# ChenyangLEI/All-In-One-Deflicker

Hardware: NVIDIA H100
Metric: atlas_iters_per_sec (higher is better)
Workload: dtype fp32 (2-term fp16 split on wgmma, fp32 accumulate)

## Files before the change

all-in-one-deflicker_b200/csrc/mlp_tc.cu:

```cuda
#include <mutex>
#include <vector>

#include "tc_api.cuh"
#include "tc_ptx.cuh"
#include "loss_math.h"

namespace b200 {
using namespace ptx;

constexpr int TM = 128;
constexpr int HID = 256;
constexpr int ITEM_BYTES = 16384;
constexpr int CHUNK_BYTES = 4 * ITEM_BYTES;
constexpr float S_ACT = 16.0f;
constexpr float S_W = 256.0f;
constexpr int ATOM_BYTES = TM * 128;
constexpr int TILE_IMG_BYTES = 4 * ATOM_BYTES;
constexpr int PE_COLS = 40;

__host__ __device__ __forceinline__ int atom_off(int m, int k) {
  const int r = m & 7;
  return (m >> 3) * 1024 + r * 128 + (((k >> 3) ^ r) << 4) + ((k & 7) << 1);
}
__host__ __device__ __forceinline__ int item_off(int n, int k) {
// ... 209 lines not shown
                                              uint32_t& scale, int& pending, const Consumer& c) {
  consume_item<NST, NN>(pp, acc, a_hi, a_lo, true, scale, pending, c);
  consume_item<NST, NN>(pp, acc, a_hi + 64, a_lo + 64, true, scale, pending, c);
  consume_item<NST, NN>(pp, acc, a_hi, a_lo, false, scale, pending, c);
  consume_item<NST, NN>(pp, acc, a_hi + 64, a_lo + 64, false, scale, pending, c);
}
template <int NST, int R>
__device__ __forceinline__ void finish_pass(Pipe<NST>& pp, float (&acc)[R], int& pending, const Consumer& c) {
  wgmma_wait<0>();
  acc_fence(acc);
  if (pending >= 0 && c.warp_leader) mbar_arrive(&pp.empty[pending]);
  pending = -1;
}

__device__ __forceinline__ void store_tile_rows(const Consumer& c, const char* a_tile, char* g_img, int64_t term_stride) {
  if (!c.leader) return;
#pragma unroll
  for (int term = 0; term < 2; ++term)
#pragma unroll
    for (int j = 0; j < 4; ++j)
      bulk_s2g(g_img + term * term_stride + j * ATOM_BYTES + c.g * WG_ROW_BYTES,
               a_tile + term * TILE_IMG_BYTES + j * ATOM_BYTES + c.g * WG_ROW_BYTES, WG_ROW_BYTES);
  bulk_commit();
}
__device__ __forceinline__ void a_tile_reusable(const Consumer& c) {
  if (c.leader) bulk_wait_read0();
  c.sync();
}
__device__ __forceinline__ void a_tile_written(const Consumer& c) {
  fence_proxy_async_smem();
  c.sync();
}

__device__ __forceinline__ uint32_t relu_flag(float v) { return (uint32_t)(-(int)__float_as_uint(v)) >> 31; }

__device__ __forceinline__ uint32_t piece_bits(uint32_t f0, uint32_t f1, int col) {
  const int i = col & 15;
  uint32_t b = (f0 << (15 - i)) | (f1 << (14 - i));
  return b;
}
__device__ __forceinline__ uint32_t quad_or(uint32_t b) {
  b |= __shfl_xor_sync(0xffffffffu, b, 1);
  b |= __shfl_xor_sync(0xffffffffu, b, 2);
  return b;
}
__device__ __forceinline__ float quad_sum(float v) {
  v += __shfl_xor_sync(0xffffffffu, v, 1);
  return v + __shfl_xor_sync(0xffffffffu, v, 2);
}

constexpr int SMEM_A = 2 * TILE_IMG_BYTES;
constexpr int SMEM_AUX = 2 * ATOM_BYTES;
constexpr int RSUM_B_BYTES = 64 * 16;
constexpr int BWD_ACC_FLOATS = 5 * 256 + 768;
constexpr int SMEM_BWD_CONST_FLOATS = CONSUMER_WGS * (RSUM_B_BYTES / 4 + BWD_ACC_FLOATS);
constexpr int SMEM_BARS = 256;
constexpr int SMEM_MAX = 227 * 1024;
template <bool ATLAS, bool BWD> struct KCfg {
  static constexpr int NST = BWD ? 5 : (ATLAS ? 3 : 5);
  static constexpr int SMEM = SMEM_A + NST * ITEM_BYTES + (ATLAS && !BWD ? SMEM_AUX : 0) +
                              (BWD ? SMEM_BWD_CONST_FLOATS * 4 : FWD_CST_BYTES) + SMEM_BARS;
  static_assert(SMEM <= SMEM_MAX, "fused kernel exceeds the shared memory of one CTA");
  static_assert(SMEM + ITEM_BYTES > SMEM_MAX, "one more weight slot would fit");
  static_assert(2 * NST * 8 + 8 <= SMEM_BARS, "ring and constant barriers exceed their shared-memory slot");
};

template <int NST>
struct SmemMap {
  char* a_tile; char* stage; char* aux; float* cst;
  uint64_t* full; uint64_t* empty;
  __device__ __forceinline__ void init(char* raw, int aux_bytes, int cst_floats) {
    char* p = raw;
    a_tile = p; p += SMEM_A;
    stage = p; p += NST * ITEM_BYTES;
    aux = p; p += aux_bytes;
    cst = reinterpret_cast<float*>(p); p += cst_floats * 4;
    full = reinterpret_cast<uint64_t*>(p);
    empty = full + NST;
  }
};

template <int NST>
__device__ __forceinline__ void setup_cta(SmemMap<NST>& sm, bool cst_bar = false) {
  if (threadIdx.x == 0) {
    if (smem_u32(sm.a_tile) & 1023u) __trap();
    for (int i = 0; i < NST; ++i) { mbar_init(&sm.full[i], 1); mbar_init(&sm.empty[i], EMPTY_ARRIVALS); }
    if (cst_bar) mbar_init(&sm.empty[NST], 1);
    fence_barrier_init();
  }
  __syncthreads();
}
constexpr int BAR_CONSUMERS = 9;

struct FwdParams {
  const float* x;
  float* y;
  const float* params;
  int64_t w_off[B200_MAX_LAYERS], b_off[B200_MAX_LAYERS];
  NetImages img;
  int cap, n_groups; const int* n_valid;
  int g_fwd, g_bwd;
  float in_scale, in_shift;
  int store_images;
  int tanh_out;
  int pe_freqs;
};

template <bool ATLAS, int NL = (ATLAS ? 8 : 6), int VAR = 0>
__global__ void __launch_bounds__(TC_THREADS, 1) tc_fwd_kernel(const __grid_constant__ FwdParams P) {
  extern __shared__ __align__(1024) char smem_raw[];
  constexpr int NST = KCfg<ATLAS, false>::NST;
  SmemMap<NST> sm; sm.init(smem_raw, ATLAS ? SMEM_AUX : 0, FWD_CST_BYTES / 4);
  const int warp = warp_uniform(), lane = threadIdx.x & 31;
  constexpr int L = NL;
  constexpr int FIRST_TC = ATLAS ? 0 : 1;
  constexpr int LAST_TC = L - 2;
  constexpr bool PE3 = ATLAS && VAR > 0;
  constexpr bool SKIPS = ATLAS && !PE3;
  constexpr int OUT = ATLAS ? (PE3 ? VAR : 3) : 2;
  constexpr int KLAST = SKIPS ? 296 : 256;
  constexpr FwdConsts CST = fwd_consts(L, !ATLAS, OUT, KLAST);
  static_assert(CST.floats * 4 <= FWD_CST_BYTES, "forward constants exceed their shared-memory slot");
  uint64_t* cst_full = &sm.empty[NST];
  const int pe_cols = VAR == 1 ? 30 : 6 * P.pe_freqs;
  setup_cta(sm, true);
  TileIter ti; ti.init(P.cap, P.n_groups, P.n_valid, P.g_fwd, P.g_bwd);

  if (warp >= CONSUMER_WGS * 4) {
    setmaxnreg_dec<PRODUCER_REGS>();
    if (warp == CONSUMER_WGS * 4 && lane == 0) {
      mbar_expect_tx(cst_full, CST.floats * 4);
      bulk_g2s(sm.cst, P.img.cst, CST.floats * 4, cst_full);
      Pipe<NST> pp{sm.full, sm.empty, sm.stage, 0};
      for (int t = blockIdx.x; t < ti.total; t += gridDim.x)
        for (int l = FIRST_TC; l <= LAST_TC; ++l) {
          const char* base = P.img.w_fwd + P.img.w_fwd_layer[l];
          if (ATLAS && l == 0) { produce_items(pp, base, 4); continue; }
          if (SKIPS && l == 4) produce_items(pp, base + (int64_t)4 * CHUNK_BYTES, 4);
          produce_items(pp, base, 16);
        }
    }
    return;
  }
  setmaxnreg_inc<CONSUMER_REGS>();
  Consumer c; c.init();
  Pipe<NST> pp{sm.full, sm.empty, sm.stage, 0};
  int pending = -1;
  const float inv_scale = 1.0f / S_W;
  const float* wlast = sm.cst + CST.wl;
  const uint32_t a_rows = smem_u32(sm.a_tile) + c.g * WG_ROW_BYTES;
  const uint32_t aux_rows = smem_u32(sm.aux) + c.g * WG_ROW_BYTES;
  float acc[128];
  mbar_wait(cst_full, 0);
  for (int t = blockIdx.x; t < ti.total; t += gridDim.x) {
    const int gt = ti.global_tile(t);
    const int64_t row0 = (int64_t)gt * TM + c.m0;
    uint16_t* bits_row = reinterpret_cast<uint16_t*>(P.img.bits) + row0 * 16;
    auto put = [&](int m, int col, float v0, float v1) {
      uint32_t h, lo;
      split2_packed(v0, v1, h, lo);
      const int off = tile_off(m, col);
      *reinterpret_cast<uint32_t*>(sm.a_tile + off) = h;
      *reinterpret_cast<uint32_t*>(sm.a_tile + TILE_IMG_BYTES + off) = lo;
    };
    uint32_t held0 = 0, held1 = 0;
    auto flags_out = [&](int slot, int i, int col, uint32_t b0, uint32_t b1) {
      if ((i & 1) == 0) { held0 = b0; held1 = b1; return; }
      b0 = quad_or(b0 | held0); b1 = quad_or(b1 | held1);
      if (P.store_images && c.q == 0) {
        uint16_t* dst = bits_row + (int64_t)slot * P.img.rows * 16 + (col >> 4);
        dst[0] = (uint16_t)b0;
        dst[8 * 16] = (uint16_t)b1;
      }
    };
    auto bias_relu = [&](const float* bias, int i, int col, float (&v)[4]) {
      const float2 bs = *reinterpret_cast<const float2*>(bias + col);
      v[0] = fmaxf(__fmaf_rn(acc[4 * i], inv_scale, bs.x), 0.f);
      v[1] = fmaxf(__fmaf_rn(acc[4 * i + 1], inv_scale, bs.y), 0.f);
      v[2] = fmaxf(__fmaf_rn(acc[4 * i + 2], inv_scale, bs.x), 0.f);
      v[3] = fmaxf(__fmaf_rn(acc[4 * i + 3], inv_scale, bs.y), 0.f);
    };
    if (ATLAS) {
      c.sync();
      for (int task = c.tid; task < 64 * 8; task += 128) {
        const int m = 64 * c.g + (task & 63), c8 = task >> 6;
        const int64_t row = (int64_t)gt * TM + m;
        float in[3] = {0.f, 0.f, 0.f};
// ... 142 lines not shown
  if (c.leader) bulk_wait_all0();
}

struct BwdParams {
  const float* dy;
  const float* y;
  const float* x;
  float* d_in;
  const float* params;
  float* grads;
  int64_t w_off[B200_MAX_LAYERS], b_off[B200_MAX_LAYERS];
  NetImages img;
  int cap, n_groups; const int* n_valid;
  int* gmax_bits;
  int g_fwd, g_bwd;
  float in_scale;
  int d_in_accumulate;
  int tanh_out;
};

__device__ __forceinline__ void grad_scales(const int* gmax_bits, bool mapping, float& s_g, float& inv_sg) {
  const float mx = __int_as_float(gmax_bits[mapping ? 1 : 0]);
  int e = 0;
  if (mx > 0.f && mx < 3.0e38f) frexpf(mx, &e);
  e = max(-60, min(60, e));
  s_g = ldexpf(1.0f, 13 - e);
  inv_sg = ldexpf(1.0f, e - 13);
}

template <bool ATLAS, int NL = (ATLAS ? 8 : 6), int VAR = 0>
__global__ void __launch_bounds__(TC_THREADS, 1) tc_bwd_kernel(const __grid_constant__ BwdParams P) {
  extern __shared__ __align__(1024) char smem_raw[];
  constexpr int NST = KCfg<ATLAS, true>::NST;
  SmemMap<NST> sm; sm.init(smem_raw, 0, SMEM_BWD_CONST_FLOATS);
  const int warp = warp_uniform(), lane = threadIdx.x & 31;
  constexpr int L = NL;
  constexpr bool PE3 = ATLAS && VAR > 0;
  constexpr bool SKIPS = ATLAS && !PE3;
  constexpr int OUT = ATLAS ? (PE3 ? VAR : 3) : 2;
  constexpr int KLAST = SKIPS ? 296 : 256;
  constexpr int LOW = 1;
  constexpr bool HAS_DPE = ATLAS && !PE3;
  constexpr bool MAPPING = OUT == 2;
  static_assert((L - 1) * 256 + (ATLAS ? 0 : 768) <= BWD_ACC_FLOATS, "gradient accumulators exceed their slice");
  char* rsum_b = reinterpret_cast<char*>(sm.cst);
  float* s_acc = sm.cst + CONSUMER_WGS * RSUM_B_BYTES / 4;
  for (int i = threadIdx.x; i < CONSUMER_WGS * BWD_ACC_FLOATS; i += blockDim.x) s_acc[i] = 0.f;
  setup_cta(sm);
  TileIter ti; ti.init(P.cap, P.n_groups, P.n_valid, P.g_fwd, P.g_bwd);
  float s_g, inv_sg;
  grad_scales(P.gmax_bits, MAPPING, s_g, inv_sg);

  if (warp >= CONSUMER_WGS * 4) {
    setmaxnreg_dec<PRODUCER_REGS>();
    if (warp == CONSUMER_WGS * 4 && lane == 0) {
      Pipe<NST> pp{sm.full, sm.empty, sm.stage, 0};
      for (int t = blockIdx.x; t < ti.total; t += gridDim.x)
        for (int l = L - 2; l >= (HAS_DPE ? 0 : LOW); --l)
          produce_items(pp, P.img.w_bwd + P.img.w_bwd_layer[l], 16, l == 0 ? 64 * 64 : ITEM_BYTES);
    }
    return;
  }
  setmaxnreg_inc<CONSUMER_REGS>();
  Consumer c; c.init();
  Pipe<NST> pp{sm.full, sm.empty, sm.stage, 0};
  int pending = -1;
  const float inv_dgrad = inv_sg * (1.0f / S_W);
  const uint16_t* bits16 = reinterpret_cast<const uint16_t*>(P.img.bits);
  const float* wlast = P.params + P.w_off[L - 1];
  const uint32_t a_rows = smem_u32(sm.a_tile) + c.g * WG_ROW_BYTES;
  const uint32_t b_rows = smem_u32(rsum_b) + c.g * RSUM_B_BYTES;
  float* g_acc = s_acc + c.g * BWD_ACC_FLOATS;
  float acc[128];
  auto row_sums = [&](int slot) {
    float (&red)[16] = *reinterpret_cast<float(*)[16]>(&acc);
    uint32_t a_base = a_rows, b_base = b_rows;
    asm volatile("" : "+r"(a_base), "+r"(b_base));
    const uint64_t ad = make_desc(a_base, ATOM_BYTES, 1024), bd = make_desc_rows16(b_base);
    wgmma_fence();
#pragma unroll
    for (int blk = 0; blk < 4; ++blk)
#pragma unroll
      for (int ks = 0; ks < 4; ++ks) {
        const uint64_t a = ad + ((blk * ATOM_BYTES + ks * 2048) >> 4), b = bd + ((ks * 256) >> 4);
        float (&d)[4] = *reinterpret_cast<float(*)[4]>(&red[4 * blk]);
        wgmma_n8<1, 1>(d, a, b, ks > 0 ? 1u : 0u);
        wgmma_n8<1, 1>(d, a + (TILE_IMG_BYTES >> 4), b, 1u);
      }
    wgmma_commit();
    wgmma_wait<0>();
    acc_fence(red);
    const bool w0 = !ATLAS && slot == 0;
    if (c.q == 0 || w0) {
#pragma unroll
      for (int blk = 0; blk < 4; ++blk)
#pragma unroll
        for (int rr = 0; rr < 2; ++rr) {
          const int n = 64 * blk + 16 * c.w4 + (c.lane >> 2) + 8 * rr;
          const float v = (red[4 * blk + 2 * rr] + red[4 * blk + 2 * rr + 1]) * inv_sg;
          if (c.q == 0) g_acc[slot * 256 + n] += v;
          else g_acc[(L - 1) * 256 + n * 3 + c.q - 1] += v * (1.0f / S_ACT);
        }
    }
  };
  auto put = [&](int m, int col, float v0, float v1) {
    uint32_t h, lo;
    split2_packed(__fmul_rn(v0, s_g), __fmul_rn(v1, s_g), h, lo);
    const int off = tile_off(m, col);
    *reinterpret_cast<uint32_t*>(sm.a_tile + off) = h;
    *reinterpret_cast<uint32_t*>(sm.a_tile + TILE_IMG_BYTES + off) = lo;
  };
  for (int t = blockIdx.x; t < ti.total; t += gridDim.x) {
    const int gt = ti.global_tile(t);
    const int64_t row0 = (int64_t)gt * TM + c.m0;
    float dzl[2][OUT];
#pragma unroll
    for (int rr = 0; rr < 2; ++rr)
#pragma unroll
      for (int jj = 0; jj < OUT; ++jj) {
        const int64_t row = row0 + 8 * rr;
        const float yv = P.y[row * OUT + jj];
        dzl[rr][jj] = P.dy[row * OUT + jj] * (P.tanh_out ? (1.0f - yv * yv) : 1.0f);
      }
#pragma unroll
    for (int jj = 0; jj < OUT; ++jj) {
      float sj = c.q == 0 ? dzl[0][jj] + dzl[1][jj] : 0.f;
#pragma unroll
      for (int o = 16; o > 0; o >>= 1) sj += __shfl_xor_sync(0xffffffffu, sj, o);
      if (lane == 0 && sj != 0.f) atomicAdd(P.grads + P.b_off[L - 1] + jj, sj);
    }
    if (c.q == 0) {
#pragma unroll
      for (int rr = 0; rr < 2; ++rr) {
        const int m = c.m0 + 8 * rr;
        uint32_t h0, l0, h1 = 0, l1 = 0;
        split2_f16(dzl[rr][0] * s_g, OUT > 1 ? dzl[rr][OUT > 1 ? 1 : 0] * s_g : 0.f, h0, l0);
        if (OUT == 3) split2_f16(dzl[rr][OUT - 1] * s_g, 0.f, h1, l1);
        char* g_hi = P.img.dzl + (int64_t)gt * ATOM_BYTES;
        char* g_lo = g_hi + P.img.w64_term_stride;
        const int r = m & 7;
        const int base = (m >> 3) * 1024 + r * 128;
#pragma unroll
        for (int c16 = 0; c16 < 8; ++c16) {
          const int off = base + ((c16 ^ r) << 4);
          *reinterpret_cast<uint4*>(g_hi + off) = c16 == 0 ? make_uint4(h0, h1, 0, 0) : make_uint4(0, 0, 0, 0);
          *reinterpret_cast<uint4*>(g_lo + off) = c16 == 0 ? make_uint4(l0, l1, 0, 0) : make_uint4(0, 0, 0, 0);
        }
      }
    }
    a_tile_reusable(c);
    if (c.tid < 64) {
      uint4 b = make_uint4(0x3C00u, 0u, 0u, 0u);
      if (!ATLAS) {
        const float4 xv = *reinterpret_cast<const float4*>(P.x + ((int64_t)gt * TM + 64 * c.g + c.tid) * 4);
        __half h, lo;
        split_f16(xv.x * S_ACT, h, lo); b.y = pack2(h, lo);
        split_f16(xv.y * S_ACT, h, lo); b.z = pack2(h, lo);
        split_f16(xv.z * S_ACT, h, lo); b.w = pack2(h, lo);
      }
      *reinterpret_cast<uint4*>(rsum_b + c.g * RSUM_B_BYTES + c.tid * 16) = b;
    }
#pragma unroll
    for (int i = 0; i < 32; ++i) {
      const int col = 8 * i + 2 * c.q;
      const uint32_t bits0 = bits16[((int64_t)(L - 2) * P.img.rows + row0) * 16 + (col >> 4)];
      const uint32_t bits1 = bits16[((int64_t)(L - 2) * P.img.rows + row0 + 8) * 16 + (col >> 4)];
      float v[4];
#pragma unroll
      for (int e = 0; e < 2; ++e) {
        float a0 = 0.f, a1 = 0.f;
#pragma unroll
        for (int jj = 0; jj < OUT; ++jj) {
          const float w = __ldg(wlast + jj * KLAST + col + e);
          a0 = fmaf(dzl[0][jj], w, a0);
          a1 = fmaf(dzl[1][jj], w, a1);
        }
        const int sh = 15 - ((col + e) & 15);
        v[e] = ((bits0 >> sh) & 1u) ? a0 : 0.f;
        v[2 + e] = ((bits1 >> sh) & 1u) ? a1 : 0.f;
      }
      put(c.m0, col, v[0], v[1]);
      put(c.m0 + 8, col, v[2], v[3]);
    }
    a_tile_written(c);
    store_tile_rows(c, sm.a_tile, P.img.dz + (int64_t)(L - 2) * P.img.slot_stride + (int64_t)gt * TILE_IMG_BYTES,
                    P.img.term_stride);
    row_sums(L - 2);
#pragma unroll 1
    for (int l = L - 2; l >= LOW; --l) {
      uint32_t scale = 0u;
      for (int kc = 0; kc < 4; ++kc)
        consume_chunk<NST, 256>(pp, acc, a_rows + kc * ATOM_BYTES, a_rows + TILE_IMG_BYTES + kc * ATOM_BYTES, scale,
                                pending, c);
      finish_pass(pp, acc, pending, c);
      const int slot = l - 1;
      const bool need_img = ATLAS || slot >= 1;
      a_tile_reusable(c);
#pragma unroll
      for (int i = 0; i < 32; ++i) {
        const int col = 8 * i + 2 * c.q;
        const uint32_t bits0 = bits16[((int64_t)slot * P.img.rows + row0) * 16 + (col >> 4)];
        const uint32_t bits1 = bits16[((int64_t)slot * P.img.rows + row0 + 8) * 16 + (col >> 4)];
        const int sh = 15 - (col & 15);
        float v[4];
        v[0] = ((bits0 >> sh) & 1u) ? __fmul_rn(acc[4 * i], inv_dgrad) : 0.f;
        v[1] = ((bits0 >> (sh - 1)) & 1u) ? __fmul_rn(acc[4 * i + 1], inv_dgrad) : 0.f;
        v[2] = ((bits1 >> sh) & 1u) ? __fmul_rn(acc[4 * i + 2], inv_dgrad) : 0.f;
        v[3] = ((bits1 >> (sh - 1)) & 1u) ? __fmul_rn(acc[4 * i + 3], inv_dgrad) : 0.f;
        put(c.m0, col, v[0], v[1]);
        put(c.m0 + 8, col, v[2], v[3]);
      }
      a_tile_written(c);
      if (need_img)
        store_tile_rows(c, sm.a_tile, P.img.dz + (int64_t)slot * P.img.slot_stride + (int64_t)gt * TILE_IMG_BYTES,
                        P.img.term_stride);
      row_sums(slot);
    }
    if (HAS_DPE) {
      float (&acc64)[32] = *reinterpret_cast<float(*)[32]>(&acc);
      uint32_t scale = 0u;
      for (int kc = 0; kc < 4; ++kc)
        consume_chunk<NST, 64>(pp, acc64, a_rows + kc * ATOM_BYTES, a_rows + TILE_IMG_BYTES + kc * ATOM_BYTES, scale,
                               pending, c);
      finish_pass(pp, acc64, pending, c);
      const char* pe_hi = P.img.pe + (int64_t)gt * ATOM_BYTES;
      const char* pe_lo = pe_hi + P.img.w64_term_stride;
      float din[2][2] = {{0.f, 0.f}, {0.f, 0.f}};
#pragma unroll
      for (int i = 0; i < 5; ++i) {
#pragma unroll
        for (int e = 0; e < 2; ++e) {
          const int col = 8 * i + 2 * c.q + e;
          const int k = col >> 2, ee = col & 3;
          const int pcol = (ee < 2) ? col + 2 : col - 2;
          const float bk = pe_freq(k);
#pragma unroll
          for (int rr = 0; rr < 2; ++rr) {
            const float g = __fmul_rn(acc64[4 * i + 2 * rr + e], inv_dgrad);
            const int off = atom_off(c.m0 + 8 * rr, pcol);
            const float partner = (__half2float(*reinterpret_cast<const __half*>(pe_hi + off)) +
                                   __half2float(*reinterpret_cast<const __half*>(pe_lo + off))) * (1.0f / S_ACT);
            din[rr][e] += (ee < 2) ? g * partner * bk : -g * partner * bk;
          }
        }
      }
      float mx = 0.f;
#pragma unroll
      for (int rr = 0; rr < 2; ++rr) {
        const float d0 = quad_sum(din[rr][0]), d1 = quad_sum(din[rr][1]);
        if (c.q == 0 && P.d_in) {
          float2* dst = reinterpret_cast<float2*>(P.d_in + (row0 + 8 * rr) * 2);
          float2 cur = P.d_in_accumulate ? *dst : make_float2(0.f, 0.f);
          cur.x += P.in_scale * d0;
          cur.y += P.in_scale * d1;
          *dst = cur;
          mx = fmaxf(mx, fmaxf(fabsf(cur.x), fabsf(cur.y)));
        }
      }
#pragma unroll
      for (int o = 16; o > 0; o >>= 1) mx = fmaxf(mx, __shfl_xor_sync(0xffffffffu, mx, o));
      if (lane == 0 && mx > 0.f) atomicMax(P.gmax_bits + 1, __float_as_int(mx));
    }
  }
  if (c.leader) bulk_wait_all0();
  named_bar(BAR_CONSUMERS, CONSUMERS);
  static_assert(CONSUMER_WGS == 2, "the flush sums two slices");
  for (int i = threadIdx.x; i < (L - 1) * 256; i += CONSUMERS) {
    const float v = s_acc[i] + s_acc[BWD_ACC_FLOATS + i];
    if (v != 0.f) atomicAdd(P.grads + P.b_off[i >> 8] + (i & 255), v);
  }
  if (!ATLAS)
    for (int i = threadIdx.x; i < 768; i += CONSUMERS) {
      const float v = s_acc[(L - 1) * 256 + i] + s_acc[BWD_ACC_FLOATS + (L - 1) * 256 + i];
      if (v != 0.f) atomicAdd(P.grads + P.w_off[0] + i, v);
    }
}

struct WgradItem {
  const char* a_img;
  const char* b_img;
  int64_t a_term, b_term;
  float* out; int ld_out;
  int a_cols;
  int b_cols;
  int transposed;
  int n_rows, n_cols;
  int cap, n_groups;
  int split, n_split;
  int mapping;
  int g_fwd, g_bwd;
};
// ... 208 lines not shown
};

static int g_wg_clusters[64];

static int ensure_attrs() {
  static bool done_dev[64] = {};
  int dev = 0;
  B200_CHECK_CUDA(cudaGetDevice(&dev));
  B200_REQUIRE(dev >= 0 && dev < 64, "device ordinal %d out of range", dev);
  bool& done = done_dev[dev];
  if (done) return B200_OK;
  for (const NetKernels& k : g_kernels) {
    B200_CHECK_CUDA(cudaFuncSetAttribute(k.fwd, cudaFuncAttributeMaxDynamicSharedMemorySize, k.fwd_smem));
    B200_CHECK_CUDA(cudaFuncSetAttribute(k.bwd, cudaFuncAttributeMaxDynamicSharedMemorySize, k.bwd_smem));
  }
  B200_CHECK_CUDA(cudaFuncSetAttribute(tc_wgrad_kernel, cudaFuncAttributeMaxDynamicSharedMemorySize, WG_SMEM));
  cudaLaunchConfig_t cfg = {};
  cfg.gridDim = dim3(WG_CLUSTER); cfg.blockDim = dim3(WG_THREADS); cfg.dynamicSmemBytes = WG_SMEM;
  B200_CHECK_CUDA(cudaOccupancyMaxActiveClusters(&g_wg_clusters[dev], tc_wgrad_kernel, &cfg));
  B200_REQUIRE(g_wg_clusters[dev] > 0, "the weight-gradient kernel's %d-CTA clusters do not fit on device %d", WG_CLUSTER, dev);
  done = true;
  return B200_OK;
}

static int launch_fwd(TcNet net, const FwdParams& P, int tiles, cudaStream_t st) {
  const NetKernels& k = g_kernels[(int)net - 1];
  k.fwd<<<min(sm_count(), tiles), TC_THREADS, k.fwd_smem, st>>>(P);
  B200_CHECK_LAUNCH();
  return B200_OK;
}

static int launch_bwd(TcNet net, const BwdParams& P, int tiles, cudaStream_t st) {
  const NetKernels& k = g_kernels[(int)net - 1];
  k.bwd<<<min(sm_count(), tiles), TC_THREADS, k.bwd_smem, st>>>(P);
  B200_CHECK_LAUNCH();
  return B200_OK;
}

static FwdParams fill_fwd(const MlpShape& sh, const NetImages& im, const float* x, float* y, const float* params, int cap,
                          int groups, const int* n_valid) {
  FwdParams P{};
  P.x = x; P.y = y; P.params = params; P.img = im; P.cap = cap; P.n_groups = groups; P.n_valid = n_valid;
  P.in_scale = 0.5f; P.in_shift = 0.5f; P.store_images = 1; P.tanh_out = 1; P.g_fwd = P.g_bwd = -1; P.pe_freqs = sh.pe;
  for (int l = 0; l < sh.L; ++l) { P.w_off[l] = sh.w_off[l]; P.b_off[l] = sh.b_off[l]; }
  return P;
}

static FwdParams fill_fwd_mapping(const MlpShape& sh, const NetImages& im, const float* x, float* y, const float* params,
                                  int cap, int groups, const int* n_valid) {
  FwdParams P = fill_fwd(sh, im, x, y, params, cap, groups, n_valid);
  P.in_scale = 1.0f; P.in_shift = 0.0f;
  return P;
}

static BwdParams fill_bwd(const MlpShape& sh, const NetImages& im, const float* dy, const float* y, const float* x,
                          float* d_in, const float* params, float* grads, int cap, int groups, const int* n_valid,
                          int* gmax_bits) {
  BwdParams P{};
  P.dy = dy; P.y = y; P.x = x; P.d_in = d_in; P.params = params; P.grads = grads; P.img = im;
  P.cap = cap; P.n_groups = groups; P.n_valid = n_valid; P.gmax_bits = gmax_bits;
  P.in_scale = 0.5f; P.d_in_accumulate = 1; P.tanh_out = 1; P.g_fwd = P.g_bwd = -1;
  for (int l = 0; l < sh.L; ++l) { P.w_off[l] = sh.w_off[l]; P.b_off[l] = sh.b_off[l]; }
  return P;
}

static void add_prep(PrepJobs& pj, const float* W, int ldw, int n_rows, int k0, int k_cnt, int transpose, char* dst) {
// ... 171 lines not shown
    B200_REQUIRE(step_shapes_ok(s), "tensor-core path is specialised to the two stage-1 networks (6-layer mapping, "
                 "with or without positional encoding, and the atlas)");
    const TcLayout lay = layout_of(s);
    const TcNet mnet = tc_net_of(*s.ms);
    const bool atlas = s.y_atlas != nullptr;
    g_pj.n = 0;
    prep_jobs_for_net(g_pj, *s.ms, lay.map, s.params, mnet, true);
    if (atlas) prep_jobs_for_net(g_pj, *s.as, lay.atl, s.params + s.ms->total, TcNet::Atlas, true);
    if (g_pj.n > MAX_PREP_JOBS) { set_error("table overflow"); return B200_ERR_INVALID; }
    WgProto protos[32]; int np = 0;
    protos_for_net(protos, np, *s.ms, lay.map, s.grads, mnet, s.n_groups, step_g_fwd(s), step_g_bwd(s));
    if (atlas) protos_for_net(protos, np, *s.as, lay.atl, s.grads + s.ms->total, TcNet::Atlas, 3);
    g_wi.n = 0;
    apportion_items(g_wi, protos, np, s.cap);
    B200_PROPAGATE(upload(g_pj, &tab->d_prep, true, st));
    B200_PROPAGATE(upload(g_wi, &tab->d_wg, true, st));
    tab->n_prep = g_pj.n; tab->n_wg = g_wi.n;
  }
  SideStream& sd = g_side[current_device()];
  if (!sd.stream) {
    B200_CHECK_CUDA(cudaStreamCreateWithFlags(&sd.stream, cudaStreamNonBlocking));
    B200_CHECK_CUDA(cudaEventCreateWithFlags(&sd.fork, cudaEventDisableTiming));
    B200_CHECK_CUDA(cudaEventCreateWithFlags(&sd.join, cudaEventDisableTiming));
  }
  B200_CHECK_CUDA(cudaEventRecord(sd.fork, st));
  B200_CHECK_CUDA(cudaStreamWaitEvent(sd.stream, sd.fork, 0));
  tc_prep_kernel<<<tab->n_prep * 4, 128, 0, sd.stream>>>(tab->d_prep);
  B200_CHECK_LAUNCH();
  B200_CHECK_CUDA(cudaEventRecord(sd.join, sd.stream));
  sd.pending = true;
  return B200_OK;
}

int tc_step_forward(const TcStep& s, cudaStream_t st) {
  const TcLayout lay = layout_of(s);
  SideStream& sd = g_side[current_device()];
  if (!sd.pending) B200_PROPAGATE(tc_begin_step(s, st));
  B200_CHECK_CUDA(cudaStreamWaitEvent(st, sd.join, 0));
  sd.pending = false;
  FwdParams pm = fill_fwd_mapping(*s.ms, lay.map, s.x_map, s.uv, s.params, s.cap, s.n_groups, s.counters);
  pm.g_fwd = step_g_fwd(s); pm.g_bwd = step_g_bwd(s);
  timer_begin(TAG_MAP_FWD, st);
  B200_PROPAGATE(launch_fwd(tc_net_of(*s.ms), pm, s.n_groups * (s.cap / TM), st));
  timer_end(TAG_MAP_FWD, st);
  if (s.y_atlas) {
    const FwdParams pa = fill_fwd(*s.as, lay.atl, s.uv, s.y_atlas, s.params + s.ms->total, s.cap, 3, s.counters);
    timer_begin(TAG_ATLAS_FWD, st);
    B200_PROPAGATE(launch_fwd(TcNet::Atlas, pa, 3 * (s.cap / TM), st));
    timer_end(TAG_ATLAS_FWD, st);
  }
  return B200_OK;
}

static const WgradItems* g_last_wg = nullptr;
static int g_last_wg_n = 0;

int tc_debug_wgrad(long long* cycles, int* shapes, int max_ctas) {
  if (!g_last_wg) { set_error("no weight-gradient launch yet"); return -1; }
  static WgradItems host;
  if (cudaMemcpy(&host, g_last_wg, sizeof(WgradItems), cudaMemcpyDeviceToHost) != cudaSuccess) return -1;
  const int n = g_last_wg_n < max_ctas ? g_last_wg_n : max_ctas;
  for (int i = 0; i < n; ++i) {
    const WgradItem& it = host.it[i / WG_CLUSTER];
    cycles[i] = host.cycles[i];
    shapes[3 * i] = it.transposed ? it.b_cols : it.a_cols; shapes[3 * i + 1] = it.transposed ? it.a_cols : it.b_cols;
    shapes[3 * i + 2] = it.n_split;
  }
  return n;
}

static int wgrad_grid(int n_items) { return WG_CLUSTER * min(n_items, wg_clusters()); }

int tc_step_backward(const TcStep& s, cudaStream_t st) {
  const TcLayout lay = layout_of(s);
  const TcTables* tab = find_tables(step_key(s), false);
  B200_REQUIRE(tab && tab->n_wg >= 0, "tensor-core backward called before forward");
  int* gmax = const_cast<int*>(s.counters) + 3;
  if (s.y_atlas) {
    const BwdParams pa = fill_bwd(*s.as, lay.atl, s.d_y, s.y_atlas, nullptr, const_cast<float*>(s.d_uv),
                                  s.params + s.ms->total, s.grads + s.ms->total, s.cap, 3, s.counters, gmax);
    timer_begin(TAG_ATLAS_BWD, st);
    B200_PROPAGATE(launch_bwd(TcNet::Atlas, pa, 3 * (s.cap / TM), st));
// ... 174 lines not shown
```

Baseline: 633.2.

## Stream backward per-tile inputs, relu flags and PE operands through the TMA ring

The producer warp now bulk-copies each tile's y, dy, last-layer weights, x, ReLU flag bits, positional-encoding images and accumulated d_in into the shared-memory ring alongside the weight items. Consumers read these from shared memory instead of scattered global loads, and the flag bits are unpacked once per layer into registers. The aim is to take the global-memory latency of these small loads off the consumer critical path. In exchange, the ring carries more items per tile, which adds pipeline pressure, and the host now requires 16-byte-aligned operands.

```diff
diff --git a/all-in-one-deflicker_b200/csrc/mlp_tc.cu b/all-in-one-deflicker_b200/csrc/mlp_tc.cu
--- a/all-in-one-deflicker_b200/csrc/mlp_tc.cu
+++ b/all-in-one-deflicker_b200/csrc/mlp_tc.cu
@@ -265,6 +265,24 @@
   c.sync();
 }
 
+struct RowFlags {
+  uint32_t p[2][2];
+  __device__ __forceinline__ void load(const char* item, int m0, int q, int hf) {
+    asm volatile("" : "+r"(m0), "+r"(q));
+    const int s = 6 - 2 * q;
+    constexpr uint32_t M = 0x03030303u;
+#pragma unroll
+    for (int rr = 0; rr < 2; ++rr) {
+      const uint4 v = *reinterpret_cast<const uint4*>(item + (m0 + 8 * rr) * 32 + hf * 16);
+      p[rr][hf] = ((v.x >> s) & M) | (((v.y >> s) & M) << 2) | (((v.z >> s) & M) << 4) | (((v.w >> s) & M) << 6);
+    }
+  }
+  __device__ __forceinline__ bool on(int rr, int i, int e) const {
+    const int pos = 16 * ((i >> 1) & 1) + 8 * (1 - (i & 1)) + 2 * ((i >> 2) & 3) + (1 - e);
+    return (p[rr][i >> 4] >> pos) & 1u;
+  }
+};
+
 __device__ __forceinline__ uint32_t relu_flag(float v) { return (uint32_t)(-(int)__float_as_uint(v)) >> 31; }
 
 __device__ __forceinline__ uint32_t piece_bits(uint32_t f0, uint32_t f1, int col) {
@@ -287,6 +305,7 @@
 constexpr int RSUM_B_BYTES = 64 * 16;
 constexpr int BWD_ACC_FLOATS = 5 * 256 + 768;
 constexpr int SMEM_BWD_CONST_FLOATS = CONSUMER_WGS * (RSUM_B_BYTES / 4 + BWD_ACC_FLOATS);
+constexpr int FLAG_BYTES = TM * 32;
 constexpr int SMEM_BARS = 256;
 constexpr int SMEM_MAX = 227 * 1024;
 template <bool ATLAS, bool BWD> struct KCfg {
@@ -607,6 +626,11 @@
   static_assert((L - 1) * 256 + (ATLAS ? 0 : 768) <= BWD_ACC_FLOATS, "gradient accumulators exceed their slice");
   char* rsum_b = reinterpret_cast<char*>(sm.cst);
   float* s_acc = sm.cst + CONSUMER_WGS * RSUM_B_BYTES / 4;
+  constexpr int TIN_Y = TM * OUT * 4;
+  constexpr int TIN_W = 2 * TIN_Y, TIN_X = TIN_W + OUT * 1024;
+  constexpr int TIN_BYTES = TIN_X + (ATLAS ? 0 : TM * 16);
+  static_assert(TIN_BYTES <= ITEM_BYTES, "a tile's inputs exceed one ring slot");
+  auto load_din = [&]() { return HAS_DPE && P.d_in && P.d_in_accumulate; };
   for (int i = threadIdx.x; i < CONSUMER_WGS * BWD_ACC_FLOATS; i += blockDim.x) s_acc[i] = 0.f;
   setup_cta(sm);
   TileIter ti; ti.init(P.cap, P.n_groups, P.n_valid, P.g_fwd, P.g_bwd);
@@ -617,9 +641,31 @@
     setmaxnreg_dec<PRODUCER_REGS>();
     if (warp == CONSUMER_WGS * 4 && lane == 0) {
       Pipe<NST> pp{sm.full, sm.empty, sm.stage, 0};
-      for (int t = blockIdx.x; t < ti.total; t += gridDim.x)
-        for (int l = L - 2; l >= (HAS_DPE ? 0 : LOW); --l)
-          produce_items(pp, P.img.w_bwd + P.img.w_bwd_layer[l], 16, l == 0 ? 64 * 64 : ITEM_BYTES);
+      const char* bits = reinterpret_cast<const char*>(P.img.bits);
+      for (int t = blockIdx.x; t < ti.total; t += gridDim.x) {
+        const int gt = ti.global_tile(t);
+        {
+          mbar_wait(&pp.empty[pp.slot()], pp.parity() ^ 1);
+          uint64_t* full = &pp.full[pp.slot()];
+          char* dst = pp.stage + pp.slot() * ITEM_BYTES;
+          mbar_expect_tx(full, TIN_BYTES);
+          bulk_g2s(dst, P.y + (int64_t)gt * TM * OUT, TIN_Y, full);
+          bulk_g2s(dst + TIN_Y, P.dy + (int64_t)gt * TM * OUT, TIN_Y, full);
+          for (int jj = 0; jj < OUT; ++jj) bulk_g2s(dst + TIN_W + jj * 1024, P.params + P.w_off[L - 1] + jj * KLAST, 1024, full);
+          if (!ATLAS) bulk_g2s(dst + TIN_X, P.x + (int64_t)gt * TM * 4, TM * 16, full);
+          ++pp.it;
+        }
+        for (int l = L - 1; l >= LOW; --l) {
+          if (l < L - 1) produce_items(pp, P.img.w_bwd + P.img.w_bwd_layer[l], 16);
+          produce_items(pp, bits + ((int64_t)(l - 1) * P.img.rows + (int64_t)gt * TM) * 32, 1, FLAG_BYTES);
+        }
+        if (HAS_DPE) {
+          produce_items(pp, P.img.w_bwd + P.img.w_bwd_layer[0], 16, 64 * 64);
+          produce_items(pp, P.img.pe + (int64_t)gt * ATOM_BYTES, 1);
+          produce_items(pp, P.img.pe + P.img.w64_term_stride + (int64_t)gt * ATOM_BYTES, 1);
+          if (load_din()) produce_items(pp, reinterpret_cast<const char*>(P.d_in + (int64_t)gt * TM * 2), 1, TM * 8);
+        }
+      }
     }
     return;
   }
@@ -628,8 +674,23 @@
   Pipe<NST> pp{sm.full, sm.empty, sm.stage, 0};
   int pending = -1;
   const float inv_dgrad = inv_sg * (1.0f / S_W);
-  const uint16_t* bits16 = reinterpret_cast<const uint16_t*>(P.img.bits);
-  const float* wlast = P.params + P.w_off[L - 1];
+  auto take = [&](int& slot) -> const char* {
+    slot = pp.slot();
+    mbar_wait(&pp.full[slot], pp.parity());
+    ++pp.it;
+    return sm.stage + slot * ITEM_BYTES;
+  };
+  auto release = [&](int slot) {
+    __syncwarp();
+    if (c.warp_leader) mbar_arrive(&pp.empty[slot]);
+  };
+  int fl_slot = 0;
+  const char* fl_item = nullptr;
+  RowFlags fl;
+  auto flag_step = [&](int i) {
+    if (i == 0) { fl_item = take(fl_slot); fl.load(fl_item, c.m0, c.q, 0); }
+    if (i == 16) { fl.load(fl_item, c.m0, c.q, 1); release(fl_slot); }
+  };
   const uint32_t a_rows = smem_u32(sm.a_tile) + c.g * WG_ROW_BYTES;
   const uint32_t b_rows = smem_u32(rsum_b) + c.g * RSUM_B_BYTES;
   float* g_acc = s_acc + c.g * BWD_ACC_FLOATS;
@@ -675,14 +736,17 @@
   for (int t = blockIdx.x; t < ti.total; t += gridDim.x) {
     const int gt = ti.global_tile(t);
     const int64_t row0 = (int64_t)gt * TM + c.m0;
+    int tin_slot;
+    const char* tin = take(tin_slot);
+    const float* s_tin = reinterpret_cast<const float*>(tin);
     float dzl[2][OUT];
 #pragma unroll
     for (int rr = 0; rr < 2; ++rr)
 #pragma unroll
       for (int jj = 0; jj < OUT; ++jj) {
-        const int64_t row = row0 + 8 * rr;
-        const float yv = P.y[row * OUT + jj];
-        dzl[rr][jj] = P.dy[row * OUT + jj] * (P.tanh_out ? (1.0f - yv * yv) : 1.0f);
+        const int m = c.m0 + 8 * rr;
+        const float yv = s_tin[m * OUT + jj];
+        dzl[rr][jj] = s_tin[TM * OUT + m * OUT + jj] * (P.tanh_out ? (1.0f - yv * yv) : 1.0f);
       }
 #pragma unroll
     for (int jj = 0; jj < OUT; ++jj) {
@@ -714,7 +778,7 @@
     if (c.tid < 64) {
       uint4 b = make_uint4(0x3C00u, 0u, 0u, 0u);
       if (!ATLAS) {
-        const float4 xv = *reinterpret_cast<const float4*>(P.x + ((int64_t)gt * TM + 64 * c.g + c.tid) * 4);
+        const float4 xv = *reinterpret_cast<const float4*>(tin + TIN_X + (64 * c.g + c.tid) * 16);
         __half h, lo;
         split_f16(xv.x * S_ACT, h, lo); b.y = pack2(h, lo);
         split_f16(xv.y * S_ACT, h, lo); b.z = pack2(h, lo);
@@ -722,27 +786,29 @@
       }
       *reinterpret_cast<uint4*>(rsum_b + c.g * RSUM_B_BYTES + c.tid * 16) = b;
     }
-#pragma unroll
-    for (int i = 0; i < 32; ++i) {
-      const int col = 8 * i + 2 * c.q;
-      const uint32_t bits0 = bits16[((int64_t)(L - 2) * P.img.rows + row0) * 16 + (col >> 4)];
-      const uint32_t bits1 = bits16[((int64_t)(L - 2) * P.img.rows + row0 + 8) * 16 + (col >> 4)];
-      float v[4];
-#pragma unroll
-      for (int e = 0; e < 2; ++e) {
-        float a0 = 0.f, a1 = 0.f;
-#pragma unroll
-        for (int jj = 0; jj < OUT; ++jj) {
-          const float w = __ldg(wlast + jj * KLAST + col + e);
-          a0 = fmaf(dzl[0][jj], w, a0);
-          a1 = fmaf(dzl[1][jj], w, a1);
-        }
-        const int sh = 15 - ((col + e) & 15);
-        v[e] = ((bits0 >> sh) & 1u) ? a0 : 0.f;
-        v[2 + e] = ((bits1 >> sh) & 1u) ? a1 : 0.f;
-      }
-      put(c.m0, col, v[0], v[1]);
-      put(c.m0 + 8, col, v[2], v[3]);
+    {
+      const float* s_wl = reinterpret_cast<const float*>(tin + TIN_W);
+#pragma unroll
+      for (int i = 0; i < 32; ++i) {
+        flag_step(i);
+        const int col = 8 * i + 2 * c.q;
+        float v[4];
+#pragma unroll
+        for (int e = 0; e < 2; ++e) {
+          float a0 = 0.f, a1 = 0.f;
+#pragma unroll
+          for (int jj = 0; jj < OUT; ++jj) {
+            const float w = s_wl[jj * 256 + col + e];
+            a0 = fmaf(dzl[0][jj], w, a0);
+            a1 = fmaf(dzl[1][jj], w, a1);
+          }
+          v[e] = fl.on(0, i, e) ? a0 : 0.f;
+          v[2 + e] = fl.on(1, i, e) ? a1 : 0.f;
+        }
+        put(c.m0, col, v[0], v[1]);
+        put(c.m0 + 8, col, v[2], v[3]);
+      }
+      release(tin_slot);
     }
     a_tile_written(c);
     store_tile_rows(c, sm.a_tile, P.img.dz + (int64_t)(L - 2) * P.img.slot_stride + (int64_t)gt * TILE_IMG_BYTES,
@@ -760,15 +826,13 @@
       a_tile_reusable(c);
 #pragma unroll
       for (int i = 0; i < 32; ++i) {
+        flag_step(i);
         const int col = 8 * i + 2 * c.q;
-        const uint32_t bits0 = bits16[((int64_t)slot * P.img.rows + row0) * 16 + (col >> 4)];
-        const uint32_t bits1 = bits16[((int64_t)slot * P.img.rows + row0 + 8) * 16 + (col >> 4)];
-        const int sh = 15 - (col & 15);
         float v[4];
-        v[0] = ((bits0 >> sh) & 1u) ? __fmul_rn(acc[4 * i], inv_dgrad) : 0.f;
-        v[1] = ((bits0 >> (sh - 1)) & 1u) ? __fmul_rn(acc[4 * i + 1], inv_dgrad) : 0.f;
-        v[2] = ((bits1 >> sh) & 1u) ? __fmul_rn(acc[4 * i + 2], inv_dgrad) : 0.f;
-        v[3] = ((bits1 >> (sh - 1)) & 1u) ? __fmul_rn(acc[4 * i + 3], inv_dgrad) : 0.f;
+        v[0] = fl.on(0, i, 0) ? __fmul_rn(acc[4 * i], inv_dgrad) : 0.f;
+        v[1] = fl.on(0, i, 1) ? __fmul_rn(acc[4 * i + 1], inv_dgrad) : 0.f;
+        v[2] = fl.on(1, i, 0) ? __fmul_rn(acc[4 * i + 2], inv_dgrad) : 0.f;
+        v[3] = fl.on(1, i, 1) ? __fmul_rn(acc[4 * i + 3], inv_dgrad) : 0.f;
         put(c.m0, col, v[0], v[1]);
         put(c.m0 + 8, col, v[2], v[3]);
       }
@@ -785,40 +849,47 @@
         consume_chunk<NST, 64>(pp, acc64, a_rows + kc * ATOM_BYTES, a_rows + TILE_IMG_BYTES + kc * ATOM_BYTES, scale,
                                pending, c);
       finish_pass(pp, acc64, pending, c);
-      const char* pe_hi = P.img.pe + (int64_t)gt * ATOM_BYTES;
-      const char* pe_lo = pe_hi + P.img.w64_term_stride;
+      int slot_hi, slot_lo;
+      const char* pe_hi = take(slot_hi);
+      const char* pe_lo = take(slot_lo);
       float din[2][2] = {{0.f, 0.f}, {0.f, 0.f}};
+      int q = c.q, m0 = c.m0;
+      asm volatile("" : "+r"(q), "+r"(m0));
 #pragma unroll
       for (int i = 0; i < 5; ++i) {
 #pragma unroll
         for (int e = 0; e < 2; ++e) {
-          const int col = 8 * i + 2 * c.q + e;
+          const int col = 8 * i + 2 * q + e;
           const int k = col >> 2, ee = col & 3;
           const int pcol = (ee < 2) ? col + 2 : col - 2;
           const float bk = pe_freq(k);
 #pragma unroll
           for (int rr = 0; rr < 2; ++rr) {
             const float g = __fmul_rn(acc64[4 * i + 2 * rr + e], inv_dgrad);
-            const int off = atom_off(c.m0 + 8 * rr, pcol);
+            const int off = atom_off(m0 + 8 * rr, pcol);
             const float partner = (__half2float(*reinterpret_cast<const __half*>(pe_hi + off)) +
                                    __half2float(*reinterpret_cast<const __half*>(pe_lo + off))) * (1.0f / S_ACT);
             din[rr][e] += (ee < 2) ? g * partner * bk : -g * partner * bk;
           }
         }
       }
+      release(slot_hi);
+      release(slot_lo);
+      int din_slot = 0;
+      const float* s_din = load_din() ? reinterpret_cast<const float*>(take(din_slot)) : nullptr;
       float mx = 0.f;
 #pragma unroll
       for (int rr = 0; rr < 2; ++rr) {
         const float d0 = quad_sum(din[rr][0]), d1 = quad_sum(din[rr][1]);
         if (c.q == 0 && P.d_in) {
-          float2* dst = reinterpret_cast<float2*>(P.d_in + (row0 + 8 * rr) * 2);
-          float2 cur = P.d_in_accumulate ? *dst : make_float2(0.f, 0.f);
+          float2 cur = load_din() ? *reinterpret_cast<const float2*>(s_din + (c.m0 + 8 * rr) * 2) : make_float2(0.f, 0.f);
           cur.x += P.in_scale * d0;
           cur.y += P.in_scale * d1;
-          *dst = cur;
+          *reinterpret_cast<float2*>(P.d_in + (row0 + 8 * rr) * 2) = cur;
           mx = fmaxf(mx, fmaxf(fabsf(cur.x), fabsf(cur.y)));
         }
       }
+      if (load_din()) release(din_slot);
 #pragma unroll
       for (int o = 16; o > 0; o >>= 1) mx = fmaxf(mx, __shfl_xor_sync(0xffffffffu, mx, o));
       if (lane == 0 && mx > 0.f) atomicMax(P.gmax_bits + 1, __float_as_int(mx));
@@ -1093,6 +1164,8 @@
 
 static int launch_bwd(TcNet net, const BwdParams& P, int tiles, cudaStream_t st) {
   const NetKernels& k = g_kernels[(int)net - 1];
+  for (const void* p : {(const void*)P.y, (const void*)P.dy, (const void*)P.x, (const void*)P.d_in, (const void*)P.params})
+    B200_REQUIRE(reinterpret_cast<uintptr_t>(p) % 16 == 0, "tensor-core backward operand %p is not 16-byte aligned", p);
   k.bwd<<<min(sm_count(), tiles), TC_THREADS, k.bwd_smem, st>>>(P);
   B200_CHECK_LAUNCH();
   return B200_OK;
```

After: 648.4 (median of 6 runs). +2.4%, better.

## Split mapping forward tail onto side stream to overlap with atlas forward

Applied to the files above, without the earlier changes.

The mapping-network forward kernel now takes a tile range. When the atlas forward follows, the main launch handles all tiles except a small leftover wave, and a second small launch on the side stream processes that tail. The atlas forward starts on the main stream right after the bulk launch and can overlap with the tail, which targets idle SMs during the mapping kernel's last partial wave. In exchange it adds an extra launch plus event synchronization, and correctness depends on the atlas forward not reading the tail tiles' outputs.

```diff
diff --git a/all-in-one-deflicker_b200/csrc/mlp_tc.cu b/all-in-one-deflicker_b200/csrc/mlp_tc.cu
--- a/all-in-one-deflicker_b200/csrc/mlp_tc.cu
+++ b/all-in-one-deflicker_b200/csrc/mlp_tc.cu
@@ -333,6 +333,7 @@
   NetImages img;
   int cap, n_groups; const int* n_valid;
   int g_fwd, g_bwd;
+  int split_grid, split_rest, split_keep, split_side;
   float in_scale, in_shift;
   int store_images;
   int tanh_out;
@@ -358,6 +359,14 @@
   const int pe_cols = VAR == 1 ? 30 : 6 * P.pe_freqs;
   setup_cta(sm, true);
   TileIter ti; ti.init(P.cap, P.n_groups, P.n_valid, P.g_fwd, P.g_bwd);
+  int t_begin = 0, t_end = ti.total;
+  if (OUT == 2 && P.split_grid > 0) {
+    const int rest = ti.total % P.split_grid;
+    int keep = 0;
+    for (int g = 0; g < P.split_keep; ++g) keep += ti.group_tiles(g);
+    const int cut = rest <= P.split_rest ? max(keep, ti.total - rest) : ti.total;
+    if (P.split_side) t_begin = cut; else t_end = cut;
+  }
 
   if (warp >= CONSUMER_WGS * 4) {
     setmaxnreg_dec<PRODUCER_REGS>();
@@ -365,7 +374,7 @@
       mbar_expect_tx(cst_full, CST.floats * 4);
       bulk_g2s(sm.cst, P.img.cst, CST.floats * 4, cst_full);
       Pipe<NST> pp{sm.full, sm.empty, sm.stage, 0};
-      for (int t = blockIdx.x; t < ti.total; t += gridDim.x)
+      for (int t = t_begin + blockIdx.x; t < t_end; t += gridDim.x)
         for (int l = FIRST_TC; l <= LAST_TC; ++l) {
           const char* base = P.img.w_fwd + P.img.w_fwd_layer[l];
           if (ATLAS && l == 0) { produce_items(pp, base, 4); continue; }
@@ -385,7 +394,7 @@
   const uint32_t aux_rows = smem_u32(sm.aux) + c.g * WG_ROW_BYTES;
   float acc[128];
   mbar_wait(cst_full, 0);
-  for (int t = blockIdx.x; t < ti.total; t += gridDim.x) {
+  for (int t = t_begin + blockIdx.x; t < t_end; t += gridDim.x) {
     const int gt = ti.global_tile(t);
     const int64_t row0 = (int64_t)gt * TM + c.m0;
     uint16_t* bits_row = reinterpret_cast<uint16_t*>(P.img.bits) + row0 * 16;
@@ -1330,22 +1339,37 @@
   return B200_OK;
 }
 
+static int step_side_ctas() { return max(1, sm_count() / 10); }
+
 int tc_step_forward(const TcStep& s, cudaStream_t st) {
   const TcLayout lay = layout_of(s);
   SideStream& sd = g_side[current_device()];
   if (!sd.pending) B200_PROPAGATE(tc_begin_step(s, st));
   B200_CHECK_CUDA(cudaStreamWaitEvent(st, sd.join, 0));
   sd.pending = false;
+  const TcNet mnet = tc_net_of(*s.ms);
+  const int map_tiles = s.n_groups * (s.cap / TM);
   FwdParams pm = fill_fwd_mapping(*s.ms, lay.map, s.x_map, s.uv, s.params, s.cap, s.n_groups, s.counters);
   pm.g_fwd = step_g_fwd(s); pm.g_bwd = step_g_bwd(s);
+  const bool side = s.y_atlas != nullptr;
+  if (side) { pm.split_grid = min(sm_count(), map_tiles); pm.split_rest = step_side_ctas(); pm.split_keep = 3; }
   timer_begin(TAG_MAP_FWD, st);
-  B200_PROPAGATE(launch_fwd(tc_net_of(*s.ms), pm, s.n_groups * (s.cap / TM), st));
-  timer_end(TAG_MAP_FWD, st);
-  if (s.y_atlas) {
+  B200_PROPAGATE(launch_fwd(mnet, pm, map_tiles, st));
+  if (side) {
+    B200_CHECK_CUDA(cudaEventRecord(sd.fork, st));
+    B200_CHECK_CUDA(cudaStreamWaitEvent(sd.stream, sd.fork, 0));
+    FwdParams pr = pm;
+    pr.split_side = 1;
+    B200_PROPAGATE(launch_fwd(mnet, pr, min(map_tiles, step_side_ctas()), sd.stream));
+    timer_end(TAG_MAP_FWD, sd.stream);
+    B200_CHECK_CUDA(cudaEventRecord(sd.join, sd.stream));
     const FwdParams pa = fill_fwd(*s.as, lay.atl, s.uv, s.y_atlas, s.params + s.ms->total, s.cap, 3, s.counters);
     timer_begin(TAG_ATLAS_FWD, st);
     B200_PROPAGATE(launch_fwd(TcNet::Atlas, pa, 3 * (s.cap / TM), st));
     timer_end(TAG_ATLAS_FWD, st);
+    B200_CHECK_CUDA(cudaStreamWaitEvent(st, sd.join, 0));
+  } else {
+    timer_end(TAG_MAP_FWD, st);
   }
   return B200_OK;
 }
```

New measurement: 634.5 before, 645.2 after (median of 6 runs). 1.02x the previous value.

## Stage backward ReLU flags, output rows and last-layer weights via TMA bulk loads

Applied to the files above, without the earlier changes.

In the atlas backward kernel, the producer warp now bulk-copies each layer's activation bitmask tile, the dy/y rows and (once per CTA) the output-layer weights into shared memory, using dedicated mbarrier pipelines. Consumers read these from shared memory instead of issuing scattered global loads inside their inner loops. To make room, the weight ring drops from five stages to four, which reduces how far weight prefetching can run ahead.

```diff
diff --git a/all-in-one-deflicker_b200/csrc/mlp_tc.cu b/all-in-one-deflicker_b200/csrc/mlp_tc.cu
--- a/all-in-one-deflicker_b200/csrc/mlp_tc.cu
+++ b/all-in-one-deflicker_b200/csrc/mlp_tc.cu
@@ -287,15 +287,24 @@
 constexpr int RSUM_B_BYTES = 64 * 16;
 constexpr int BWD_ACC_FLOATS = 5 * 256 + 768;
 constexpr int SMEM_BWD_CONST_FLOATS = CONSUMER_WGS * (RSUM_B_BYTES / 4 + BWD_ACC_FLOATS);
+constexpr int FLAG_BYTES = TM * 32;
+constexpr int FLAG_STAGES = 2;
+constexpr int ROW_IN_BYTES = TM * 3 * 2 * 4;
+constexpr int BWD_WLAST_BYTES = 3 * 256 * 4;
+constexpr int SMEM_BWD_STAGE = FLAG_STAGES * FLAG_BYTES + ROW_IN_BYTES + BWD_WLAST_BYTES;
+constexpr int BWD_SIDE_BARS = 2 * FLAG_STAGES + 2;
 constexpr int SMEM_BARS = 256;
 constexpr int SMEM_MAX = 227 * 1024;
 template <bool ATLAS, bool BWD> struct KCfg {
-  static constexpr int NST = BWD ? 5 : (ATLAS ? 3 : 5);
-  static constexpr int SMEM = SMEM_A + NST * ITEM_BYTES + (ATLAS && !BWD ? SMEM_AUX : 0) +
-                              (BWD ? SMEM_BWD_CONST_FLOATS * 4 : FWD_CST_BYTES) + SMEM_BARS;
+  static constexpr bool STAGED = BWD && ATLAS;
+  static constexpr int NST = BWD ? (STAGED ? 4 : 5) : (ATLAS ? 3 : 5);
+  static constexpr int AUX = STAGED ? SMEM_BWD_STAGE : (ATLAS && !BWD ? SMEM_AUX : 0);
+  static constexpr int SMEM = SMEM_A + NST * ITEM_BYTES + AUX + (BWD ? SMEM_BWD_CONST_FLOATS * 4 : FWD_CST_BYTES) +
+                              SMEM_BARS;
   static_assert(SMEM <= SMEM_MAX, "fused kernel exceeds the shared memory of one CTA");
   static_assert(SMEM + ITEM_BYTES > SMEM_MAX, "one more weight slot would fit");
-  static_assert(2 * NST * 8 + 8 <= SMEM_BARS, "ring and constant barriers exceed their shared-memory slot");
+  static_assert(2 * NST * 8 + (STAGED ? BWD_SIDE_BARS : 1) * 8 <= SMEM_BARS,
+                "ring and side barriers exceed their shared-memory slot");
 };
 
 template <int NST>
@@ -594,7 +603,8 @@
 __global__ void __launch_bounds__(TC_THREADS, 1) tc_bwd_kernel(const __grid_constant__ BwdParams P) {
   extern __shared__ __align__(1024) char smem_raw[];
   constexpr int NST = KCfg<ATLAS, true>::NST;
-  SmemMap<NST> sm; sm.init(smem_raw, 0, SMEM_BWD_CONST_FLOATS);
+  constexpr bool STAGED = KCfg<ATLAS, true>::STAGED;
+  SmemMap<NST> sm; sm.init(smem_raw, KCfg<ATLAS, true>::AUX, SMEM_BWD_CONST_FLOATS);
   const int warp = warp_uniform(), lane = threadIdx.x & 31;
   constexpr int L = NL;
   constexpr bool PE3 = ATLAS && VAR > 0;
@@ -608,18 +618,58 @@
   char* rsum_b = reinterpret_cast<char*>(sm.cst);
   float* s_acc = sm.cst + CONSUMER_WGS * RSUM_B_BYTES / 4;
   for (int i = threadIdx.x; i < CONSUMER_WGS * BWD_ACC_FLOATS; i += blockDim.x) s_acc[i] = 0.f;
+  char* s_flags = sm.aux;
+  float* s_rows = reinterpret_cast<float*>(sm.aux + FLAG_STAGES * FLAG_BYTES);
+  constexpr int Y_OFF = TM * OUT;
+  static_assert(2 * Y_OFF * 4 <= ROW_IN_BYTES, "row inputs exceed their staging buffer");
+  float* s_wlast = reinterpret_cast<float*>(sm.aux + FLAG_STAGES * FLAG_BYTES + ROW_IN_BYTES);
+  static_assert(OUT * 256 * 4 <= BWD_WLAST_BYTES, "output-layer weights exceed their staging buffer");
+  if (STAGED)
+    for (int i = threadIdx.x; i < OUT * 256; i += blockDim.x)
+      s_wlast[i] = P.params[P.w_off[L - 1] + (i >> 8) * KLAST + (i & 255)];
+  uint64_t* side = &sm.empty[NST];
+  if (STAGED && threadIdx.x == 0) {
+    for (int i = 0; i < FLAG_STAGES; ++i) { mbar_init(&side[i], 1); mbar_init(&side[FLAG_STAGES + i], EMPTY_ARRIVALS); }
+    mbar_init(&side[2 * FLAG_STAGES], 1);
+    mbar_init(&side[2 * FLAG_STAGES + 1], EMPTY_ARRIVALS);
+  }
   setup_cta(sm);
   TileIter ti; ti.init(P.cap, P.n_groups, P.n_valid, P.g_fwd, P.g_bwd);
   float s_g, inv_sg;
   grad_scales(P.gmax_bits, MAPPING, s_g, inv_sg);
+  Pipe<FLAG_STAGES> fp{side, side + FLAG_STAGES, s_flags, 0};
+  Pipe<1> rp{side + 2 * FLAG_STAGES, side + 2 * FLAG_STAGES + 1, reinterpret_cast<char*>(s_rows), 0};
 
   if (warp >= CONSUMER_WGS * 4) {
     setmaxnreg_dec<PRODUCER_REGS>();
     if (warp == CONSUMER_WGS * 4 && lane == 0) {
       Pipe<NST> pp{sm.full, sm.empty, sm.stage, 0};
-      for (int t = blockIdx.x; t < ti.total; t += gridDim.x)
-        for (int l = L - 2; l >= (HAS_DPE ? 0 : LOW); --l)
+      auto produce_flags = [&](int gt, int slot) {
+        mbar_wait(&fp.empty[fp.slot()], fp.parity() ^ 1);
+        mbar_expect_tx(&fp.full[fp.slot()], FLAG_BYTES);
+        bulk_g2s(fp.stage + fp.slot() * FLAG_BYTES, P.img.bits + ((int64_t)slot * P.img.rows + (int64_t)gt * TM) * 8,
+                 FLAG_BYTES, &fp.full[fp.slot()]);
+        ++fp.it;
+      };
+      auto produce_rows = [&](int gt) {
+        constexpr uint32_t YB = TM * OUT * 4;
+        const int64_t r0 = (int64_t)gt * TM;
+        mbar_wait(&rp.empty[0], rp.parity() ^ 1);
+        mbar_expect_tx(&rp.full[0], P.tanh_out ? 2 * YB : YB);
+        bulk_g2s(s_rows, P.dy + r0 * OUT, YB, &rp.full[0]);
+        if (P.tanh_out) bulk_g2s(s_rows + Y_OFF, P.y + r0 * OUT, YB, &rp.full[0]);
+        ++rp.it;
+      };
+      if (STAGED && blockIdx.x < ti.total) produce_rows(ti.global_tile(blockIdx.x));
+      for (int t = blockIdx.x; t < ti.total; t += gridDim.x) {
+        const int gt = ti.global_tile(t);
+        if (STAGED) produce_flags(gt, L - 2);
+        for (int l = L - 2; l >= (HAS_DPE ? 0 : LOW); --l) {
+          if (STAGED && l >= 1) produce_flags(gt, l - 1);
           produce_items(pp, P.img.w_bwd + P.img.w_bwd_layer[l], 16, l == 0 ? 64 * 64 : ITEM_BYTES);
+          if (STAGED && l == L - 2 && t + (int)gridDim.x < ti.total) produce_rows(ti.global_tile(t + gridDim.x));
+        }
+      }
     }
     return;
   }
@@ -628,8 +678,6 @@
   Pipe<NST> pp{sm.full, sm.empty, sm.stage, 0};
   int pending = -1;
   const float inv_dgrad = inv_sg * (1.0f / S_W);
-  const uint16_t* bits16 = reinterpret_cast<const uint16_t*>(P.img.bits);
-  const float* wlast = P.params + P.w_off[L - 1];
   const uint32_t a_rows = smem_u32(sm.a_tile) + c.g * WG_ROW_BYTES;
   const uint32_t b_rows = smem_u32(rsum_b) + c.g * RSUM_B_BYTES;
   float* g_acc = s_acc + c.g * BWD_ACC_FLOATS;
@@ -672,17 +720,39 @@
     *reinterpret_cast<uint32_t*>(sm.a_tile + off) = h;
     *reinterpret_cast<uint32_t*>(sm.a_tile + TILE_IMG_BYTES + off) = lo;
   };
+  const uint16_t* bits16 = reinterpret_cast<const uint16_t*>(P.img.bits);
+  auto flags_wait = [&]() -> const uint16_t* {
+    mbar_wait(&fp.full[fp.slot()], fp.parity());
+    return reinterpret_cast<const uint16_t*>(fp.stage + fp.slot() * FLAG_BYTES) + c.m0 * 16;
+  };
+  auto flag_word = [&](const uint16_t* fl, int slot, int64_t row, int r8, int col) -> uint32_t {
+    if constexpr (STAGED) return fl[r8 * 16 + (col >> 4)];
+    else return bits16[((int64_t)slot * P.img.rows + row + r8) * 16 + (col >> 4)];
+  };
+  auto release = [&](auto& pipe) {
+    if (!STAGED) return;
+    __syncwarp();
+    if (c.warp_leader) mbar_arrive(&pipe.empty[pipe.slot()]);
+    ++pipe.it;
+  };
   for (int t = blockIdx.x; t < ti.total; t += gridDim.x) {
     const int gt = ti.global_tile(t);
     const int64_t row0 = (int64_t)gt * TM + c.m0;
+    if (STAGED) mbar_wait(&rp.full[0], rp.parity());
     float dzl[2][OUT];
 #pragma unroll
     for (int rr = 0; rr < 2; ++rr)
 #pragma unroll
       for (int jj = 0; jj < OUT; ++jj) {
-        const int64_t row = row0 + 8 * rr;
-        const float yv = P.y[row * OUT + jj];
-        dzl[rr][jj] = P.dy[row * OUT + jj] * (P.tanh_out ? (1.0f - yv * yv) : 1.0f);
+        if constexpr (STAGED) {
+          const int m = c.m0 + 8 * rr;
+          const float yv = P.tanh_out ? s_rows[Y_OFF + m * OUT + jj] : 0.f;
+          dzl[rr][jj] = s_rows[m * OUT + jj] * (P.tanh_out ? (1.0f - yv * yv) : 1.0f);
+        } else {
+          const int64_t row = row0 + 8 * rr;
+          const float yv = P.y[row * OUT + jj];
+          dzl[rr][jj] = P.dy[row * OUT + jj] * (P.tanh_out ? (1.0f - yv * yv) : 1.0f);
+        }
       }
 #pragma unroll
     for (int jj = 0; jj < OUT; ++jj) {
@@ -701,7 +771,9 @@
         char* g_hi = P.img.dzl + (int64_t)gt * ATOM_BYTES;
         char* g_lo = g_hi + P.img.w64_term_stride;
         const int r = m & 7;
-        const int base = (m >> 3) * 1024 + r * 128;
+        int base = (m >> 3) * 1024 + r * 128;
+        if (ATLAS) asm volatile("" : "+r"(base));
+
 #pragma unroll
         for (int c16 = 0; c16 < 8; ++c16) {
           const int off = base + ((c16 ^ r) << 4);
@@ -722,18 +794,20 @@
       }
       *reinterpret_cast<uint4*>(rsum_b + c.g * RSUM_B_BYTES + c.tid * 16) = b;
     }
+    release(rp);
+    const uint16_t* fl = STAGED ? flags_wait() : nullptr;
 #pragma unroll
     for (int i = 0; i < 32; ++i) {
       const int col = 8 * i + 2 * c.q;
-      const uint32_t bits0 = bits16[((int64_t)(L - 2) * P.img.rows + row0) * 16 + (col >> 4)];
-      const uint32_t bits1 = bits16[((int64_t)(L - 2) * P.img.rows + row0 + 8) * 16 + (col >> 4)];
+      const uint32_t bits0 = flag_word(fl, L - 2, row0, 0, col);
+      const uint32_t bits1 = flag_word(fl, L - 2, row0, 8, col);
       float v[4];
 #pragma unroll
       for (int e = 0; e < 2; ++e) {
         float a0 = 0.f, a1 = 0.f;
 #pragma unroll
         for (int jj = 0; jj < OUT; ++jj) {
-          const float w = __ldg(wlast + jj * KLAST + col + e);
+          const float w = STAGED ? s_wlast[jj * 256 + col + e] : __ldg(P.params + P.w_off[L - 1] + jj * KLAST + col + e);
           a0 = fmaf(dzl[0][jj], w, a0);
           a1 = fmaf(dzl[1][jj], w, a1);
         }
@@ -744,6 +818,7 @@
       put(c.m0, col, v[0], v[1]);
       put(c.m0 + 8, col, v[2], v[3]);
     }
+    release(fp);
     a_tile_written(c);
     store_tile_rows(c, sm.a_tile, P.img.dz + (int64_t)(L - 2) * P.img.slot_stride + (int64_t)gt * TILE_IMG_BYTES,
                     P.img.term_stride);
@@ -758,11 +833,12 @@
       const int slot = l - 1;
       const bool need_img = ATLAS || slot >= 1;
       a_tile_reusable(c);
+      const uint16_t* fl = STAGED ? flags_wait() : nullptr;
 #pragma unroll
       for (int i = 0; i < 32; ++i) {
         const int col = 8 * i + 2 * c.q;
-        const uint32_t bits0 = bits16[((int64_t)slot * P.img.rows + row0) * 16 + (col >> 4)];
-        const uint32_t bits1 = bits16[((int64_t)slot * P.img.rows + row0 + 8) * 16 + (col >> 4)];
+        const uint32_t bits0 = flag_word(fl, slot, row0, 0, col);
+        const uint32_t bits1 = flag_word(fl, slot, row0, 8, col);
         const int sh = 15 - (col & 15);
         float v[4];
         v[0] = ((bits0 >> sh) & 1u) ? __fmul_rn(acc[4 * i], inv_dgrad) : 0.f;
@@ -772,6 +848,7 @@
         put(c.m0, col, v[0], v[1]);
         put(c.m0 + 8, col, v[2], v[3]);
       }
+      release(fp);
       a_tile_written(c);
       if (need_img)
         store_tile_rows(c, sm.a_tile, P.img.dz + (int64_t)slot * P.img.slot_stride + (int64_t)gt * TILE_IMG_BYTES,
```

After: 638.5 before, 640.6 after (median of 6 runs). About the same (+0.3%).
